# andimarafioti/faster-qwen3-tts

Measured on AMD Instinct MI355X. Metric: real-time factor (audio s / wall s), Qwen3-TTS-12Hz-0.6B voice-clone streaming chunk_size=8; p50 TTFA in ttfa_ms_p50, higher is better.
Workload: dtype bf16

## Files before the change

faster-qwen3-tts_amd/csrc/fq3_api.hip:

```cpp
#define FQ3_SKINNY_EXTERN
#include "fq3_ctx.h"
#include "sampler.cuh"
#include "sampler_wave.cuh"
#include "skinny_gemm.cuh"
#include "state_kernels.cuh"

#include <cstdio>
#include <cstdlib>
#include <cstring>
#include <map>
#include <string>
#include <type_traits>
#include <vector>

using namespace fq3;

static thread_local std::string g_err;
static int fail(int code, const std::string& m) { g_err = m; return code; }
int fq3_fail_(int code, const std::string& m) { return fail(code, m); }
#define HIPCHK(x) do { hipError_t e_ = (x); if (e_ != hipSuccess) return fail(FQ3_EHIP, std::string(#x) + ": " + hipGetErrorString(e_)); } while (0)

extern "C" const char* fq3_last_error(void) { return g_err.c_str(); }
extern "C" void fq3_set_error_(const char* msg) { g_err = msg ? msg : ""; }
extern "C" int fq3_abi_version(void) { return FQ3_ABI_VERSION; }
// ... 160 lines not shown
    };
    int r;
    {
        StackBufs& b = c->tk;
        b.max_seq = cfg->max_seq_len;
        b.max_blocks = (cfg->max_seq_len + kKeysPerTile - 1) / kKeysPerTile;
        b.workers = std::min(kMaxWorkers, b.max_blocks);
        if (!pool) {
            if ((r = pool_create_(cfg, b.max_blocks, &pool))) return r;
            pool->is_private = true;
        }
        b.pool = pool;
        { std::lock_guard<std::mutex> lk(pool->mu); ++pool->users; }
        b.k = pool->k; b.v = pool->v;
        if ((r = dmalloc(c, (void**)&b.d_table, (size_t)b.max_blocks * sizeof(int)))) return r;
        if (pool->is_private && (r = kv_ensure(c, cfg->max_seq_len, nullptr, true))) return r;
    }
    if ((r = alloc_stack(c->pk, p, pred_seq))) return r;
    const int Hm = std::max(t.hidden, p.hidden), Im = std::max(t.inter, p.inter);
    const int qkvm = std::max(t.n_heads + 2 * t.n_kv_heads, p.n_heads + 2 * p.n_kv_heads) * kHeadDim;
    const int Vm = std::max(t.vocab, p.vocab);
    const int G = cfg->num_code_groups;
    const int frames = cfg->max_frames > 0 ? cfg->max_frames : 4096;
    c->cfg.max_frames = frames;
    if ((r = dmalloc(c, &c->h, (size_t)Hm * c->esz))) return r;
    if ((r = dmalloc(c, &c->h2, (size_t)Hm * c->esz))) return r;
    if ((r = dmalloc(c, &c->qkv2, (size_t)qkvm * c->esz))) return r;
    if ((r = dmalloc(c, &c->attn_out, (size_t)qkvm * c->esz))) return r;
    if ((r = dmalloc(c, &c->attn_out2, (size_t)qkvm * c->esz))) return r;
    if ((r = dmalloc(c, &c->act2, (size_t)Im * c->esz))) return r;
    if ((r = dmalloc(c, &c->pred_x2, (size_t)p.hidden * c->esz))) return r;
    if ((r = dmalloc(c, &c->xin, (size_t)Hm * c->esz))) return r;
    if ((r = dmalloc(c, &c->tmp_hidden, (size_t)Hm * c->esz))) return r;
    if ((r = dmalloc(c, &c->qkv, (size_t)qkvm * c->esz))) return r;
    if ((r = dmalloc(c, &c->act, (size_t)Im * c->esz))) return r;
    if ((r = dmalloc(c, &c->logits, (size_t)Vm * c->esz))) return r;
    if ((r = dmalloc(c, &c->past_hidden, (size_t)t.hidden * c->esz))) return r;
    if ((r = dmalloc(c, &c->ph_hold, (size_t)t.hidden * c->esz))) return r;
    if ((r = dmalloc(c, &c->pred_in, (size_t)2 * t.hidden * c->esz))) return r;
    if ((r = dmalloc(c, &c->pred_next, (size_t)t.hidden * c->esz))) return r;
    if ((r = dmalloc(c, &c->pred_x, (size_t)p.hidden * c->esz))) return r;
    if ((r = dmalloc(c, &c->plogits, (size_t)(G - 1) * p.vocab * c->esz))) return r;
    const int maxkv = std::max(t.n_kv_heads, p.n_kv_heads);
    c->part_stride = (size_t)maxkv * kMaxWorkers * 4 * kPartStride;
    if ((r = dmalloc(c, (void**)&c->part, 2 * c->part_stride * sizeof(float)))) return r;
    if ((r = dmalloc(c, (void**)&c->rope_now, 2 * 64 * sizeof(float)))) return r;
    if ((r = dmalloc(c, (void**)&c->seen_api, kMaxVocab))) return r;
    if ((r = dmalloc(c, (void**)&c->st, sizeof(DecodeState)))) return r;
    if ((r = dmalloc(c, (void**)&c->seen, kMaxVocab))) return r;
    if ((r = dmalloc(c, (void**)&c->codes, (size_t)(frames + 1) * G * sizeof(int)))) return r;
    if ((r = dmalloc(c, (void**)&c->ids64, (size_t)64 * sizeof(int64_t)))) return r;
    if ((r = dmalloc(c, (void**)&c->d_pemb, (size_t)64 * sizeof(void*)))) return r;
    HIPCHK(hipStreamCreateWithFlags(&c->cap_stream, hipStreamNonBlocking));
    return FQ3_OK;
}

extern "C" int fq3_set_option(fq3_ctx* c, const char* key, int value) {
    if (!c || !key) return fail(FQ3_EINVAL, "null argument");
    const std::string k(key);
    if (k == "weight_nt") c->opt_nt = value;
    else if (k == "pred_m2") c->opt_m2 = value;
    else if (k == "pred_attn") c->opt_pred_attn = value;
    else if (k == "rows_per_wave_max") c->opt_rmax = value;
    else if (k == "prefill_mode") c->prefill_mode = value;
    else if (k == "flash_prefill") c->opt_flash_prefill = value;
    else if (k == "flash_small") c->opt_flash_small = value;
    else if (k == "cont_pack") c->opt_cont_pack = value;
    else if (k == "swiglu_tile") c->opt_swiglu_tile = value;
    else if (k == "packed_weights") c->opt_packed = value;
    else if (k == "skinny_gemm") c->opt_no_skinny = !value;
    else return fail(FQ3_EINVAL, "unknown option: " + k);
    fq3_graph_reset(c);
    return FQ3_OK;
}

extern "C" int fq3_graph_reset(fq3_ctx* c) {
    if (!c) return fail(FQ3_EINVAL, "null ctx");
    if (c->exec) { (void)hipGraphExecDestroy(c->exec); c->exec = nullptr; }
    if (c->graph) { (void)hipGraphDestroy(c->graph); c->graph = nullptr; }
    return FQ3_OK;
}

namespace {
struct PackedEntry { void* p; int refs; int N, K; };
std::mutex g_packed_mu;
std::map<std::pair<const void*, int>, PackedEntry> g_packed;
}
const void* fq3_packed_find_(const void* W, int kind) {
    std::lock_guard<std::mutex> lk(g_packed_mu);
    auto it = g_packed.find({W, kind});
    return it == g_packed.end() ? nullptr : it->second.p;
}
int fq3_packed_acquire_(const void* W, int N, int K, int kind) {
    if (!W || !skinny_pack_ok(N, K) || (kind == 1 && (N / 2) % 8) || (kind == 2 && N % 512)) return FQ3_EUNSUPPORTED;
    std::lock_guard<std::mutex> lk(g_packed_mu);
    auto it = g_packed.find({W, kind});
    if (it != g_packed.end()) {
        if (it->second.N != N || it->second.K != K) return fail(FQ3_EINVAL, "a matrix is bound with two different shapes");
        ++it->second.refs;
        return FQ3_OK;
    }
    void* p = nullptr;
    if (hipMalloc(&p, (size_t)N * K * 2) != hipSuccess) { (void)hipGetLastError(); return fail(FQ3_ENOMEM, "no device memory for the fragment-major weight copy"); }
    skinny_pack(reinterpret_cast<const bf16_t*>(W), reinterpret_cast<bf16_t*>(p), N, K, kind == 1 ? N / 2 : (kind == 2 ? -(N / 2) : 0), nullptr);
    if (hipStreamSynchronize(nullptr) != hipSuccess) { (void)hipFree(p); return fail(FQ3_EHIP, "packing a weight matrix failed"); }
    g_packed[{W, kind}] = PackedEntry{p, 1, N, K};
    return FQ3_OK;
}
void fq3_packed_release_(const void* W, int kind) {
    std::lock_guard<std::mutex> lk(g_packed_mu);
    auto it = g_packed.find({W, kind});
    if (it == g_packed.end()) return;
    if (--it->second.refs <= 0) { (void)hipFree(it->second.p); g_packed.erase(it); }
}
static void packed_release_all(fq3_ctx* c) {
    for (auto& r : c->packed_refs) fq3_packed_release_(r.first, r.second);
    c->packed_refs.clear();
}
static int packed_acquire_all(fq3_ctx* c) {
    if (c->cfg.dtype != FQ3_BF16) return FQ3_OK;
    auto take = [&](const void* W, int N, int K, int kind) -> int {
        const int r = fq3_packed_acquire_(W, N, K, kind);
        if (r == FQ3_OK) c->packed_refs.emplace_back(W, kind);
        return r == FQ3_EUNSUPPORTED ? FQ3_OK : r;
    };
    auto stack = [&](const std::vector<fq3_layer_weights>& L, const fq3_stack_dims& d) -> int {
        const int qd = d.n_heads * kHeadDim, kvd = d.n_kv_heads * kHeadDim;
        for (const fq3_layer_weights& l : L) {
            if (int r = take(l.qkv, qd + 2 * kvd, d.hidden, 0)) return r;
            if (int r = take(l.o, d.hidden, qd, 0)) return r;
            if (int r = take(l.gate_up, 2 * d.inter, d.hidden, 1)) return r;
            if (int r = take(l.gate_up, 2 * d.inter, d.hidden, 0)) return r;
            if (int r = take(l.down, d.hidden, d.inter, 0)) return r;
        }
        return FQ3_OK;
    };
    if (int r = stack(c->tl, c->cfg.talker)) return r;
    if (int r = stack(c->pl, c->cfg.predictor)) return r;
    for (const fq3_layer_weights& l : c->tl) if (int r = take(l.gate_up, 2 * c->cfg.talker.inter, c->cfg.talker.hidden, 2)) return r;
    if (int r = take(c->wt.codec_head, c->cfg.talker.vocab, c->cfg.talker.hidden, 0)) return r;
    for (const void* h : c->lmh) if (int r = take(h, c->cfg.predictor.vocab, c->cfg.predictor.hidden, 0)) return r;
    return FQ3_OK;
}

extern "C" int fq3_ctx_destroy(fq3_ctx* c) {
    if (!c) return FQ3_OK;
    (void)hipDeviceSynchronize();
    fq3_graph_reset(c);
    packed_release_all(c);
    if (c->cap_stream) (void)hipStreamDestroy(c->cap_stream);
    if (fq3_kv_pool* p = c->tk.pool) {
        (void)fq3_kv_release(c, 0);
        bool last;
        { std::lock_guard<std::mutex> lk(p->mu); last = --p->users == 0; }
        if (p->is_private && last) pool_free_(p);
    }
    for (void* p : c->allocs) (void)hipFree(p);
    delete c;
    return FQ3_OK;
}

extern "C" int fq3_bind_weights(fq3_ctx* c, const fq3_weight_table* w) {
    if (!c || !w) return fail(FQ3_EINVAL, "null argument");
    const int G = c->cfg.num_code_groups;
    if (!w->talker_layers || !w->predictor_layers || !w->codec_embedding || !w->codec_head || !w->talker_final_norm ||
        !w->predictor_final_norm || !w->predictor_embeddings || !w->lm_heads || !w->talker_cos || !w->talker_sin ||
        !w->pred_cos || !w->pred_sin)
        return fail(FQ3_EINVAL, "weight table has null entries");
    if (c->cfg.has_projection && !w->proj_w) return fail(FQ3_EINVAL, "has_projection set but proj_w is null");
    if (w->talker_rope_len < c->cfg.max_seq_len || w->pred_rope_len < G + 1)
        return fail(FQ3_EINVAL, "rope tables shorter than the caches");
    c->wt = *w;
    c->tl.assign(w->talker_layers, w->talker_layers + c->cfg.talker.n_layers);
    c->pl.assign(w->predictor_layers, w->predictor_layers + c->cfg.predictor.n_layers);
    c->pemb.assign(w->predictor_embeddings, w->predictor_embeddings + (G - 1));
    c->lmh.assign(w->lm_heads, w->lm_heads + (G - 1));
    for (auto& l : c->tl) if (!l.qkv || !l.o || !l.gate_up || !l.down || !l.input_norm || !l.post_norm || !l.q_norm || !l.k_norm)
        return fail(FQ3_EINVAL, "talker layer has null weights");
    for (auto& l : c->pl) if (!l.qkv || !l.o || !l.gate_up || !l.down || !l.input_norm || !l.post_norm || !l.q_norm || !l.k_norm)
        return fail(FQ3_EINVAL, "predictor layer has null weights");
    HIPCHK(hipMemcpy(c->d_pemb, c->pemb.data(), (G - 1) * sizeof(void*), hipMemcpyHostToDevice));
    (void)hipDeviceSynchronize();
    packed_release_all(c);
    if (int r = packed_acquire_all(c)) { packed_release_all(c); return r; }
    c->bound = true;
    fq3_graph_reset(c);
    return FQ3_OK;
}

template <typename T, int NCH, int PRO, int EPI, bool NT, int M = 1>
static void launch_gemv_n(const GemvArgs& a, int rmax, hipStream_t s) {
    const int R = gemv_rows_per_wave<NCH, EPI>(a.N, rmax);
    const int grid = gemv_grid(a.N, R);
    const size_t shm = gemv_lds_bytes<PRO, M>(a.K);
    if constexpr (MaxRows<NCH, EPI>::v >= 2) {
        if (R == 2) { gemv_launch<T, NCH, PRO, EPI, NT, M, 2>(a, grid, shm, s); return; }
    }
    gemv_launch<T, NCH, PRO, EPI, NT, M, 1>(a, grid, shm, s);
}
template <typename T, int PRO, int EPI>
static int launch_gemv2_t(const GemvArgs& a, int rmax, hipStream_t s) {
    constexpr int most = gemv_most_chunks(PRO, 2);
    const int n = gemv_chunks(a.K, most);
// ... 722 lines not shown
}
static int enqueue_frame(fq3_ctx* c, hipStream_t s) {
    return c->cfg.dtype == FQ3_BF16 ? enqueue_frame_t<bf16_t>(c, s) : enqueue_frame_t<float>(c, s);
}

extern "C" int fq3_graph_capture(fq3_ctx* c, void* stream) {
    NEED_BOUND(c);
    if (c->exec) return FQ3_OK;
    (void)stream;
    hipStream_t cs = c->cap_stream;
    HIPCHK(hipStreamBeginCapture(cs, hipStreamCaptureModeRelaxed));
    int r = enqueue_frame(c, cs);
    hipGraph_t g = nullptr;
    hipError_t e = hipStreamEndCapture(cs, &g);
    if (r) { if (g) (void)hipGraphDestroy(g); return r; }
    if (e != hipSuccess) return fail(FQ3_EHIP, std::string("hipStreamEndCapture: ") + hipGetErrorString(e));
    c->graph = g;
    HIPCHK(hipGraphInstantiate(&c->exec, c->graph, nullptr, nullptr, 0));
    return FQ3_OK;
}

extern "C" int fq3_decode_frames(fq3_ctx* c, int n_frames, void* stream) {
    NEED_BOUND(c);
    hipStream_t s = (hipStream_t)stream;
    for (int i = 0; i < n_frames; ++i) {
        if (c->exec) { HIPCHK(hipGraphLaunch(c->exec, s)); }
        else if (int r = enqueue_frame(c, s)) return r;
    }
    LAUNCH_CHECK();
    return FQ3_OK;
}

extern "C" int fq3_decode_poll(fq3_ctx* c, int* n_frames_total, int* done, void* stream) {
    if (!c) return fail(FQ3_EINVAL, "null ctx");
    hipStream_t s = (hipStream_t)stream;
    DecodeState h;
    HIPCHK(hipMemcpyAsync(&h, c->st, sizeof h, hipMemcpyDeviceToHost, s));
    HIPCHK(hipStreamSynchronize(s));
    if (n_frames_total) *n_frames_total = h.frame;
    if (done) *done = h.done == 2 ? 2 : (h.done || h.token == h.eos_id);
    return FQ3_OK;
}

extern "C" int fq3_decode_codes(fq3_ctx* c, int from, int count, int64_t* out, void* stream) {
    if (!c || !out) return fail(FQ3_EINVAL, "null argument");
    if (from < 0 || count < 0 || from + count > c->cfg.max_frames) return fail(FQ3_EINVAL, "range");
    const int G = c->cfg.num_code_groups, n = count * G;
    if (n == 0) return FQ3_OK;
    hipLaunchKernelGGL(codes_to_i64_kernel, dim3((n + 255) / 256), dim3(256), 0, (hipStream_t)stream,
                       c->codes + (size_t)from * G, out, n);
    LAUNCH_CHECK();
    return FQ3_OK;
}
```

faster-qwen3-tts_amd/csrc/fq3_ctx.h:

```cpp
#pragma once
#include "../../include/fq3hip.h"
#include "decode_kernels.cuh"
#include <hip/hip_runtime.h>
#include <mutex>
#include <string>
#include <utility>
#include <vector>

struct fq3_kv_pool {
    int dtype = 0, esz = 2, n_layers = 0, n_kv = 0, n_blocks = 0;
    size_t blk_elems = 0;
    std::vector<void*> k, v;
    std::vector<int> free_list;
    std::mutex mu;
    int in_use_high = 0;
    int users = 0;
    bool is_private = false;
};

struct StackBufs {
    std::vector<void*> k, v;
    int max_seq = 0, workers = 1;
    fq3_kv_pool* pool = nullptr;
    int* d_table = nullptr;
    std::vector<int> blocks;
    int max_blocks = 0;
};

struct fq3_ctx {
    fq3_config cfg{};
    int esz = 2;
    std::vector<fq3_layer_weights> tl, pl;
    fq3_weight_table wt{};
    std::vector<const void*> pemb, lmh;
    const void** d_pemb = nullptr;
    bool bound = false;
    StackBufs tk, pk;
    void *h = nullptr, *xin = nullptr, *qkv = nullptr, *act = nullptr, *logits = nullptr, *past_hidden = nullptr;
    void *pred_in = nullptr, *pred_x = nullptr, *pred_next = nullptr, *plogits = nullptr, *tmp_hidden = nullptr;
    void *attn_out = nullptr, *attn_out2 = nullptr;
    void *h2 = nullptr, *qkv2 = nullptr, *act2 = nullptr, *pred_x2 = nullptr;
    size_t part_stride = 0;
    float* part = nullptr;
    float* rope_now = nullptr;
    unsigned char* seen_api = nullptr;
    fq3::DecodeState* st = nullptr;
    fq3::TeacherForcing* tf = nullptr;
    unsigned char* seen = nullptr;
    int* codes = nullptr;
    int64_t* ids64 = nullptr;
    int n_pad = 0, rope_delta = 0;
    int opt_nt = 1;
    int opt_m2 = 1;
    int opt_pred_attn = 1;
    int opt_rmax = 2;
    int opt_flash_prefill = 1;
    int opt_flash_small = 1;
    int opt_cont_pack = 1;
    int opt_swiglu_tile = 1;
    int opt_packed = 1;
    std::vector<std::pair<const void*, int>> packed_refs;
    int opt_no_skinny = 0;
    int prefill_mode = 0;
    bool talker_wave = true;
    fq3_sampling pred_sampling{0.9f, 50, 1.0f, 1, 1.0f};
    hipGraph_t graph = nullptr;
    hipGraphExec_t exec = nullptr;
    hipStream_t cap_stream = nullptr;
    std::vector<void*> allocs;
    fq3_prompt_weights pw{};
    bool pw_bound = false;
    void *pw_x = nullptr, *pw_h = nullptr;
    int pw_cap = 0;
    void* ph_hold = nullptr;
    void *tt_tab = nullptr, *tt_x = nullptr, *tt_h = nullptr;
    int tt_alloc = 0;
    int tt_cap = 0, tt_rows = 0;
    bool tt_open = false, tt_session = false;
    bool armed = false;
    const void* begin_trailing = nullptr; int begin_trailing_len = 0;
    void *pf_x = nullptr, *pf_xn = nullptr, *pf_qkv = nullptr, *pf_att = nullptr, *pf_gu = nullptr, *pf_act = nullptr, *pf_ws = nullptr;
};


const void* fq3_packed_find_(const void* W, int kind);
int fq3_packed_acquire_(const void* W, int N, int K, int kind);
void fq3_packed_release_(const void* W, int kind);

int fq3_fail_(int code, const std::string& m);
int fq3_kv_ensure_(fq3_ctx* c, int n_pos, hipStream_t s);
int fq3_prefill_reserve_(fq3_ctx* c);
int fq3_prefill_mfma_(fq3_ctx* c, const void* embeds, int L, int n_pad, void* out_logits, void* out_hidden, hipStream_t s);
int fq3_prefill_continue_mfma_(fq3_ctx* c, const void* embeds, int start, int n, void* out_logits, void* out_hidden, hipStream_t s);
int fq3_prefill_continue_batch_mfma_(fq3_ctx* const* cs, int n, const void* const* embeds, const int* start, const int* cnt,
                                     void* const* out_logits, void* const* out_hidden, hipStream_t s);
int fq3_prefill_batch_mfma_(fq3_ctx* const* cs, int n, const void* const* embeds, const int* L, const int* n_pad, void* const* out_logits,
                            void* const* out_hidden, hipStream_t s);
int fq3_codec_head_launch_(fq3_ctx* c, const void* hidden, void* out_logits, hipStream_t s);
int fq3_dmalloc_(fq3_ctx* c, void** p, size_t bytes);
void fq3_text_project_launch_(fq3_ctx* c, const int64_t* ids, int n, void* x, void* h, void* out, hipStream_t s);
```

faster-qwen3-tts_amd/csrc/state_kernels.cuh:

```cuda
#pragma once
#include "batch_kernels.cuh"

namespace fq3 {

static __global__ void poll_gather_kernel(LaneSt t, int B, int* out) {
    const int l = threadIdx.x;
    if (l < B) {
        const DecodeState* st = t.st[l];
        out[2 * l] = st->frame;
        out[2 * l + 1] = st->done == 2 ? 2 : ((st->done || st->token == st->eos_id) ? 1 : 0);
    }
}

struct AppendDst { void* dst[kMaxLanes]; int first[kMaxLanes + 1]; };
struct AppendPub { DecodeState* st[kMaxLanes]; int rows[kMaxLanes]; int closes[kMaxLanes]; };
static __global__ __launch_bounds__(256) void text_scatter_kernel(AppendDst a, int n_items, const u32x4* y, int row_vec) {
    const int r = blockIdx.x;
    int lo = 0, hi = n_items - 1;
    while (lo < hi) {
        const int mid = (lo + hi + 1) >> 1;
        if (a.first[mid] <= r) lo = mid; else hi = mid - 1;
    }
    u32x4* d = gptr(reinterpret_cast<u32x4*>(a.dst[lo])) + (size_t)(r - a.first[lo]) * row_vec;
    const u32x4* src = y + (size_t)r * row_vec;
    for (int e = threadIdx.x; e < row_vec; e += 256) d[e] = src[e];
}
static __global__ __launch_bounds__(kMaxLanes) void text_publish_lanes_kernel(AppendPub p, int n_items) {
    const int i = threadIdx.x;
    if (i < n_items) {
        DecodeState* st = gptr(p.st[i]);
        st->trailing_len = p.rows[i];
        if (p.closes[i]) st->text_open = 0;
    }
}

struct KvTableVals { int v[128]; };
static __global__ void kv_table_write_kernel(int* table, KvTableVals vals, int first, int count) {
    const int i = threadIdx.x;
    if (i < count) table[first + i] = vals.v[i];
}

template <typename T, bool TO_CACHE>
__global__ __launch_bounds__(256) void kv_paged_copy_kernel(T* cache, const int* table, int blk_stride, T* dense, int n_kv, int L) {
    constexpr int EPC = 16 / (int)sizeof(T), CPR = kHeadDim / EPC;
    const int i = blockIdx.x * 256 + threadIdx.x;
    if (i >= n_kv * L * CPR) return;
    const int ch = i % CPR, row = i / CPR, key = row % L, h = row / L;
    T* cp = cache + (size_t)table[key / kKeysPerTile] * blk_stride + ((size_t)h * kKeysPerTile + key % kKeysPerTile) * kHeadDim + ch * EPC;
    T* dp = dense + ((size_t)h * L + key) * kHeadDim + ch * EPC;
    if (TO_CACHE) *reinterpret_cast<u32x4*>(cp) = *reinterpret_cast<const u32x4*>(dp);
    else *reinterpret_cast<u32x4*>(dp) = *reinterpret_cast<const u32x4*>(cp);
}

struct KvAdoptTab { void* dst[128]; const void* src[128]; };
template <typename T>
__global__ __launch_bounds__(256) void kv_adopt_kernel(KvAdoptTab t, const int* dst_table, const int* src_table, int blk_elems) {
    const int which = blockIdx.x, b = blockIdx.y;
    const u32x4* s = reinterpret_cast<const u32x4*>(reinterpret_cast<const T*>(t.src[which]) + (size_t)src_table[b] * blk_elems);
    u32x4* d = reinterpret_cast<u32x4*>(reinterpret_cast<T*>(t.dst[which]) + (size_t)dst_table[b] * blk_elems);
    const int n16 = blk_elems * (int)sizeof(T) / 16;
    for (int i = threadIdx.x; i < n16; i += 256) d[i] = s[i];
}

static __global__ __launch_bounds__(256) void decode_arm_kernel(DecodeState* st, DecodeState init, unsigned char* seen, int seen_bytes,
                                                                uint32_t* past_hidden, const uint32_t* ph_src, int ph_words) {
    for (int i = threadIdx.x; i < seen_bytes / 4; i += 256) reinterpret_cast<uint32_t*>(seen)[i] = 0u;
    for (int i = threadIdx.x; i < ph_words; i += 256) past_hidden[i] = ph_src[i];
    if (threadIdx.x == 0) *st = init;
}
static __global__ void decode_set_forced_kernel(TeacherForcing* tf, const int* forced, int* decisions) {
    tf->forced = forced; tf->decisions = decisions;
}
static __global__ void decode_cancel_kernel(DecodeState* st) { st->done = 1; }
static __global__ void codes_to_i64_kernel(const int* src, int64_t* dst, int n) {
    const int i = blockIdx.x * blockDim.x + threadIdx.x;
    if (i < n) dst[i] = src[i];
}

}
```

faster-qwen3-tts_amd/fq3hip/_lib.py:

```python
from __future__ import annotations

import ctypes as C
import os

import torch

_HERE = os.path.dirname(os.path.abspath(__file__))
LIB_PATH = os.path.join(os.path.dirname(_HERE), "lib", "libfq3hip.so")

FQ3_BF16, FQ3_F32, FQ3_BF16X2 = 0, 1, 2
FQ3_PCM_F32, FQ3_PCM_S16, FQ3_PCM_MULAW, FQ3_PCM_ALAW = 0, 1, 2, 3
FQ3_STAGE_GROUP_MAX = 32
FQ3_OK, FQ3_EINVAL, FQ3_EHIP, FQ3_ESTATE, FQ3_ETOOLONG, FQ3_EUNSUPPORTED, FQ3_ENOMEM = 0, -1, -2, -3, -4, -5, -6

vp = C.c_void_p
i32 = C.c_int32


class StackDims(C.Structure):
    _fields_ = [("hidden", i32), ("inter", i32), ("n_layers", i32), ("n_heads", i32), ("n_kv_heads", i32),
                ("head_dim", i32), ("vocab", i32), ("rms_eps", C.c_float)]


class Config(C.Structure):
# ... 78 lines not shown


class RefEncConfig(C.Structure):
    _fields_ = [("num_filters", i32), ("n_ratios", i32), ("ratios", i32 * 8), ("kernel_size", i32), ("last_kernel_size", i32),
                ("residual_kernel_size", i32), ("n_residual_layers", i32), ("dilation_growth_rate", i32), ("compress", i32),
                ("hidden", i32), ("n_layers", i32), ("n_heads", i32), ("head_dim", i32), ("inter", i32), ("sliding_window", i32),
                ("norm_eps", C.c_float), ("num_quantizers", i32), ("num_semantic", i32), ("codebook_size", i32),
                ("codebook_dim", i32), ("max_positions", i32), ("mel_dim", i32), ("n_fft", i32), ("hop", i32),
                ("n_bins_padded", i32), ("n_enc", i32), ("enc_channels", i32 * 8), ("enc_kernel_sizes", i32 * 8),
                ("enc_dilations", i32 * 8), ("attn_channels", i32), ("res2net_scale", i32), ("se_channels", i32),
                ("enc_dim", i32)]


SIGNATURES = {
    "fq3_last_error": (C.c_char_p, []),
    "fq3_abi_version": (C.c_int, []),
    "fq3_ctx_create": (C.c_int, [C.POINTER(Config), C.POINTER(vp)]),
    "fq3_ctx_destroy": (C.c_int, [vp]),
    "fq3_kv_pool_create": (C.c_int, [C.POINTER(Config), C.c_int, C.POINTER(vp)]),
    "fq3_kv_pool_destroy": (C.c_int, [vp]),
    "fq3_kv_pool_stats": (C.c_int, [vp, C.POINTER(C.c_int), C.POINTER(C.c_int), C.POINTER(C.c_int), C.POINTER(C.c_int64)]),
    "fq3_ctx_create_pooled": (C.c_int, [C.POINTER(Config), vp, C.POINTER(vp)]),
    "fq3_kv_reserve": (C.c_int, [vp, C.c_int, vp]),
    "fq3_kv_release": (C.c_int, [vp, C.c_int]),
    "fq3_kv_blocks": (C.c_int, [vp]),
    "fq3_bind_weights": (C.c_int, [vp, C.POINTER(WeightTable)]),
    "fq3_set_option": (C.c_int, [vp, C.c_char_p, C.c_int]),
    "fq3_kv_import": (C.c_int, [vp, C.c_int, vp, vp, C.c_int, vp]),
    "fq3_kv_export": (C.c_int, [vp, C.c_int, vp, vp, C.c_int, vp]),
    "fq3_kv_adopt": (C.c_int, [vp, vp, C.c_int, vp]),
    "fq3_kv_copy": (C.c_int, [vp, vp, C.c_int, vp]),
    "fq3_set_generation_state": (C.c_int, [vp, C.c_int, C.c_int]),
    "fq3_talker_step": (C.c_int, [vp, vp, C.c_int, vp, vp]),
    "fq3_prefill": (C.c_int, [vp, vp, C.c_int, C.c_int, vp, vp, vp]),
    "fq3_prefill_continue": (C.c_int, [vp, vp, C.c_int, C.c_int, vp, vp, vp]),
    "fq3_prefill_reserve": (C.c_int, [vp]),
    "fq3_prefill_continue_batch": (C.c_int, [C.POINTER(vp), C.c_int, C.POINTER(vp), C.POINTER(C.c_int), C.POINTER(C.c_int), C.POINTER(vp),
                                             C.POINTER(vp), vp]),
    "fq3_prefill_batch": (C.c_int, [C.POINTER(vp), C.c_int, C.POINTER(vp), C.POINTER(C.c_int), C.POINTER(C.c_int), C.POINTER(vp),
                                    C.POINTER(vp), vp]),
    "fq3_set_prefill_mode": (C.c_int, [vp, C.c_int]),
    "fq3_codec_head": (C.c_int, [vp, vp, vp, vp]),
    "fq3_set_predictor_sampling": (C.c_int, [vp, C.POINTER(Sampling)]),
    "fq3_predictor_loop": (C.c_int, [vp, vp, vp, vp, vp, vp]),
    "fq3_sample": (C.c_int, [vp, vp, C.c_int, C.POINTER(Sampling), vp, C.c_int, C.c_int, C.c_int, C.c_int,
                             C.c_int, vp, vp, vp]),
    "fq3_apply_repetition_penalty": (C.c_int, [vp, vp, C.c_int, vp, C.c_int, C.c_float, vp]),
    "fq3_decode_begin": (C.c_int, [vp, C.POINTER(DecodeParams), vp]),
    "fq3_decode_cancel": (C.c_int, [vp, vp]),
    "fq3_decode_set_forced": (C.c_int, [vp, vp, vp, vp]),
    "fq3_decode_frames": (C.c_int, [vp, C.c_int, vp]),
    "fq3_decode_poll": (C.c_int, [vp, C.POINTER(C.c_int), C.POINTER(C.c_int), vp]),
    "fq3_decode_codes": (C.c_int, [vp, C.c_int, C.c_int, vp, vp]),
    "fq3_graph_capture": (C.c_int, [vp, vp]),
    "fq3_graph_reset": (C.c_int, [vp]),
    "fq3_bind_prompt_weights": (C.c_int, [vp, C.POINTER(PromptWeights)]),
    "fq3_text_project": (C.c_int, [vp, vp, C.c_int, vp, vp]),
    "fq3_decode_text_open": (C.c_int, [vp, C.c_int, vp]),
    "fq3_decode_text_append": (C.c_int, [vp, vp, C.c_int, C.c_int, vp]),
    "fq3_decode_text_rows": (C.c_int, [vp, C.POINTER(C.c_int), C.POINTER(C.c_int)]),
    "fq3_decode_text_read": (C.c_int, [vp, C.c_int, C.c_int, vp, vp]),
    "fq3_prompt_rows": (C.c_int, [vp, vp, C.c_int, vp, C.c_int, vp, C.c_int, vp, vp, vp]),
    "fq3_batch_create": (C.c_int, [C.POINTER(vp), C.c_int, C.POINTER(vp)]),
    "fq3_batch_destroy": (C.c_int, [vp]),
    "fq3_batch_size": (C.c_int, [vp]),
    "fq3_batch_frames": (C.c_int, [vp, C.c_int, vp]),
    "fq3_batch_graph_capture": (C.c_int, [vp, vp]),
    "fq3_batch_graph_reset": (C.c_int, [vp]),
    "fq3_batch_set_option": (C.c_int, [vp, C.c_char_p, C.c_int]),
    "fq3_batch_set_group_streams": (C.c_int, [vp, C.POINTER(vp), C.c_int]),
    "fq3_batch_poll_async": (C.c_int, [vp, C.c_int, vp]),
    "fq3_batch_poll_wait": (C.c_int, [vp, C.c_int, C.POINTER(C.c_int), C.POINTER(C.c_int)]),
    "fq3_batch_text_append": (C.c_int, [vp, C.c_int, C.POINTER(C.c_int32), C.POINTER(C.c_int32), C.POINTER(C.c_int32), vp, vp]),
    "fq3_codec_create": (C.c_int, [C.POINTER(CodecConfig), C.POINTER(vp)]),
    "fq3_codec_destroy": (C.c_int, [vp]),
    "fq3_codec_set_option": (C.c_int, [vp, C.c_char_p, C.c_int]),
    "fq3_codec_bind": (C.c_int, [vp, C.c_char_p, vp, C.c_int64]),
    "fq3_codec_finalize": (C.c_int, [vp, vp]),
    "fq3_codec_num_samples": (C.c_int64, [vp, C.c_int]),
    "fq3_codec_decode": (C.c_int, [vp, vp, C.c_int, vp, vp]),
    "fq3_codec_decode_tail": (C.c_int, [vp, vp, C.c_int, C.c_int64, vp, vp]),
    "fq3_codec_decode_batch": (C.c_int, [vp, vp, C.c_int, C.c_int, C.c_int64, vp, vp]),
    "fq3_codec_prefix_create": (C.c_int, [vp, vp, C.c_int, C.POINTER(vp), vp]),
    "fq3_codec_prefix_destroy": (C.c_int, [vp]),
    "fq3_codec_prefix_frames": (C.c_int, [vp]),
    "fq3_codec_decode_batch_prefix": (C.c_int, [vp, C.POINTER(vp), vp, C.c_int, C.c_int, C.c_int64, vp, vp]),
    "fq3_codec_stream_create": (C.c_int, [vp, vp, C.POINTER(vp), vp]),
    "fq3_codec_stream_reset": (C.c_int, [vp, vp, vp]),
    "fq3_codec_stream_destroy": (C.c_int, [vp]),
    "fq3_codec_stream_frames": (C.c_int, [vp]),
    "fq3_codec_stream_push": (C.c_int, [vp, C.POINTER(vp), C.c_int, vp, C.c_int, vp, vp]),
    "fq3_refenc_create": (C.c_int, [C.POINTER(RefEncConfig), C.POINTER(vp)]),
    "fq3_refenc_destroy": (C.c_int, [vp]),
    "fq3_refenc_bind": (C.c_int, [vp, C.c_char_p, vp, C.c_int64]),
    "fq3_refenc_finalize": (C.c_int, [vp, vp]),
    "fq3_refenc_num_frames": (C.c_int64, [vp, C.c_int64]),
    "fq3_refenc_encode": (C.c_int, [vp, vp, C.c_int64, vp, vp]),
    "fq3_refenc_speaker": (C.c_int, [vp, vp, C.c_int64, vp, vp, vp]),
    "fq3_audio_out_design": (C.c_int, [C.c_int, C.c_int, C.c_int, C.POINTER(C.c_int), C.POINTER(C.c_int), C.POINTER(C.c_int),
                                       C.POINTER(C.c_float), C.c_int64]),
    "fq3_audio_out_count": (C.c_int64, [C.c_int, C.c_int, C.c_int, C.c_int64, C.c_int]),
    "fq3_audio_out_create": (C.c_int, [C.POINTER(AudioOutConfig), C.POINTER(vp)]),
    "fq3_audio_out_destroy": (C.c_int, [vp]),
    "fq3_audio_out_reset": (C.c_int, [vp, vp]),
    "fq3_audio_out_push": (C.c_int, [vp, vp, C.c_int64, C.c_int, vp, C.c_int64, C.POINTER(C.c_int64), vp]),
    "fq3_tsm_design": (C.c_int, [C.c_int, C.c_int, C.POINTER(C.c_int), C.POINTER(C.c_int), C.POINTER(C.c_int),
# ... 80 lines not shown
```

faster-qwen3-tts_amd/fq3hip/engine.py:

```python
from __future__ import annotations

import ctypes as C
import threading
from typing import Dict, Optional

import torch

from . import _lib as L
from .config import TTSConfig, StackConfig

Weights = Dict[str, torch.Tensor]
_CAPTURE_LOCK = threading.Lock()


def _ptr(t: Optional[torch.Tensor]) -> Optional[int]:
    return None if t is None else t.data_ptr()


def rope_tables(head_dim: int, theta: float, n_pos: int, dtype: torch.dtype):
    inv = 1.0 / (theta ** (torch.arange(0, head_dim, 2, dtype=torch.float) / head_dim))
    ang = torch.arange(n_pos, dtype=torch.float32)[:, None] * inv[None, :]
    return ang.cos().to(dtype).float().contiguous(), ang.sin().to(dtype).float().contiguous()


# ... 429 lines not shown
        self._loop_keep = (past_hidden, trailing_text, tts_pad_embed, talker_noise, pred_noise)
        L.check(self.lib.fq3_decode_begin(self.ctx, C.byref(p), self._stream()))

    def graph_capture(self):
        with _CAPTURE_LOCK:
            L.check(self.lib.fq3_graph_capture(self.ctx, self._stream()))

    def graph_reset(self):
        L.check(self.lib.fq3_graph_reset(self.ctx))

    def decode_frames(self, n: int):
        L.check(self.lib.fq3_decode_frames(self.ctx, int(n), self._stream()))

    def decode_poll(self):
        n, d = C.c_int(0), C.c_int(0)
        L.check(self.lib.fq3_decode_poll(self.ctx, C.byref(n), C.byref(d), self._stream()))
        return n.value, bool(d.value)

    def decode_poll_state(self):
        n, d = C.c_int(0), C.c_int(0)
        L.check(self.lib.fq3_decode_poll(self.ctx, C.byref(n), C.byref(d), self._stream()))
        return n.value, int(d.value)

    def decode_text_open(self, capacity_rows: int):
        L.check(self.lib.fq3_decode_text_open(self.ctx, int(capacity_rows), self._stream()))

    def decode_text_append(self, ids, final: bool = False):
        if isinstance(ids, torch.Tensor):
            t = ids.reshape(-1).to(device=self.device, dtype=torch.long).contiguous()
        else:
            t = torch.tensor([int(i) for i in ids], dtype=torch.long, device=self.device)
        n = int(t.numel())
        L.check(self.lib.fq3_decode_text_append(self.ctx, t.data_ptr() if n else None, n, int(bool(final)), self._stream()))
        self._text_ids_keep = t

    def decode_text_rows(self):
        n, c = C.c_int(0), C.c_int(0)
        L.check(self.lib.fq3_decode_text_rows(self.ctx, C.byref(n), C.byref(c)))
        return n.value, bool(c.value)

    def decode_text_read(self, start: int = 0, count: Optional[int] = None) -> torch.Tensor:
        if count is None:
            count = self.decode_text_rows()[0] - int(start)
        out = self.new(int(count), self.cfg.talker.hidden_size)
        L.check(self.lib.fq3_decode_text_read(self.ctx, int(start), int(count), out.data_ptr(), self._stream()))
        return out

    def decode_codes(self, start: int, count: int) -> torch.Tensor:
        out = torch.empty(count, self.cfg.num_code_groups, dtype=torch.long, device=self.device)
        if count:
            L.check(self.lib.fq3_decode_codes(self.ctx, int(start), int(count), out.data_ptr(), self._stream()))
        return out

    def close(self):
        if getattr(self, "ctx", None) and self.ctx.value:
            self.lib.fq3_ctx_destroy(self.ctx)
            self.ctx = L.vp()

    def __del__(self):
        try:
            self.close()
        except Exception:
            pass


class Fq3Batch:

    def __init__(self, lanes):
        lanes = list(lanes)
        if not 1 <= len(lanes) <= 128:
            raise ValueError("a batch holds 1..128 lanes")
        self.lanes = lanes
        self.lib = lanes[0].lib
        self.device = lanes[0].device
        arr = (L.vp * len(lanes))(*[e.ctx.value for e in lanes])
        self.handle = L.vp()
        with torch.cuda.device(self.device):
            L.check(self.lib.fq3_batch_create(arr, len(lanes), C.byref(self.handle)))

    def __len__(self):
        return len(self.lanes)

    def _stream(self) -> int:
        return torch.cuda.current_stream(self.device).cuda_stream

    def frames(self, n: int):
        L.check(self.lib.fq3_batch_frames(self.handle, int(n), self._stream()))

    def graph_capture(self):
        with _CAPTURE_LOCK:
            L.check(self.lib.fq3_batch_graph_capture(self.handle, self._stream()))

    def graph_reset(self):
        L.check(self.lib.fq3_batch_graph_reset(self.handle))

    def set_option(self, key: str, value: int):
        L.check(self.lib.fq3_batch_set_option(self.handle, key.encode(), int(value)))

    def poll_async(self, slot: int):
        L.check(self.lib.fq3_batch_poll_async(self.handle, int(slot), self._stream()))

    def poll_wait(self, slot: int):
        n = len(self.lanes)
        a, d = (C.c_int * n)(), (C.c_int * n)()
        L.check(self.lib.fq3_batch_poll_wait(self.handle, int(slot), a, d))
        return list(a), [bool(x) for x in d]
# ... 37 lines not shown
```

faster-qwen3-tts_amd/fq3hip/generate.py:

```python
from __future__ import annotations

import numbers
import time
from typing import Optional, Tuple

import torch

from .predictor_graph import PredictorGraph
from .talker_graph import TalkerGraph

NOISE_RING = 64


def validate_seed(seed):
    if seed is None:
        return None
    if isinstance(seed, bool) or not isinstance(seed, numbers.Integral):
        raise ValueError(f"seed must be an integer in [0, 2**64) or None, got {type(seed).__name__}")
    seed = int(seed)
    if not 0 <= seed < 2 ** 64:
        raise ValueError(f"seed must be in [0, 2**64), got {seed}")
    return seed


def expand_seeds(seeds, n: int):
    if seeds is None:
        return [None] * n
    if isinstance(seeds, (list, tuple)):
        if len(seeds) != n:
            raise ValueError(f"seeds: {len(seeds)} entries for {n} utterances")
        return [validate_seed(s) for s in seeds]
    s = validate_seed(seeds)
    return [(s + i) % 2 ** 64 for i in range(n)]


def _refill(engine, talker_noise, pred_noise, seed=None, first_frame=0):
    if seed is not None:
        if talker_noise is not None or pred_noise is not None:
            engine.noise_fill(talker_noise, pred_noise, seed, first_frame)
        return
    if talker_noise is not None:
        talker_noise.exponential_(1)
    if pred_noise is not None:
        pred_noise.exponential_(1)


def _first_noise(eng, V, do_sample, seed):
    if not do_sample:
        return None
    if seed is not None:
        return eng.noise_first(seed)
    return torch.empty(V, dtype=eng.dtype, device=eng.device).exponential_(1)


def _n_pad_of(attention_mask) -> int:
    if attention_mask is None:
        return 0
    known = noted_n_pad(attention_mask)
    return known if known is not None else int((attention_mask[0] == 0).sum())


def noted_n_pad(attention_mask):
    note = getattr(attention_mask, "fq3_n_pad", None)
    if not (isinstance(note, tuple) and len(note) == 2):
# ... 86 lines not shown
                     trailing_text=tth, tts_pad_embed=tpe, temperature=temperature, top_k=top_k, top_p=top_p,
                     do_sample=do_sample, repetition_penalty=repetition_penalty, min_new_tokens=min_new_tokens,
                     max_new_tokens=max_frames, talker_noise=tn, pred_noise=pn, noise_frames=NOISE_RING)
    if use_graph:
        eng.graph_capture()
    else:
        eng.graph_reset()
    return eng, tn, pn, max_frames


def _prefill_and_arm(talker, talker_input_embeds, attention_mask, trailing_text_hiddens, tts_pad_embed, config,
                     predictor_graph, talker_graph, max_new_tokens, min_new_tokens, temperature, top_k, top_p,
                     do_sample, repetition_penalty, use_graph, cache=None, seed=None):
    token, hidden, n_rows, n_pad = _prefill_first_token(talker_graph.engine, talker_input_embeds, attention_mask, config,
                                                        min_new_tokens, temperature, top_k, top_p, do_sample, cache=cache, seed=seed)
    return _arm_decode(talker, config, token, hidden, n_rows, attention_mask, trailing_text_hiddens, tts_pad_embed, predictor_graph,
                       talker_graph, max_new_tokens, min_new_tokens, temperature, top_k, top_p, do_sample, repetition_penalty,
                       use_graph, n_pad=n_pad, seed=seed)


def run_frames(eng, tn, pn, issued: int, count: int, seed=None):
    while count > 0:
        if issued % NOISE_RING == 0:
            if seed is None:
                _refill(eng, tn, pn)
            else:
                _refill(eng, tn, pn, seed, issued)
        k = min(count, NOISE_RING - issued % NOISE_RING)
        eng.decode_frames(k)
        issued += k
        count -= k
    return issued


@torch.inference_mode()
def fast_generate(talker, talker_input_embeds: torch.Tensor, attention_mask: torch.Tensor,
                  trailing_text_hiddens: torch.Tensor, tts_pad_embed: torch.Tensor, config,
                  predictor_graph: PredictorGraph, talker_graph: TalkerGraph, max_new_tokens: int = 2048,
                  min_new_tokens: int = 2, temperature: float = 0.9, top_k: int = 50, top_p: float = 1.0,
                  do_sample: bool = True, repetition_penalty: float = 1.05,
                  subtalker_dosample: Optional[bool] = None, subtalker_top_k: Optional[int] = None,
                  subtalker_top_p: Optional[float] = None, subtalker_temperature: Optional[float] = None,
                  parity_mode: bool = False, poll_every: int = 8, seed: Optional[int] = None) -> Tuple[Optional[torch.Tensor], dict]:
    seed = validate_seed(seed)
    t_start = time.time()
    eng, tn, pn, max_frames = _prefill_and_arm(
        talker, talker_input_embeds, attention_mask, trailing_text_hiddens, tts_pad_embed, config, predictor_graph,
        talker_graph, max_new_tokens, min_new_tokens, temperature, top_k, top_p, do_sample, repetition_penalty,
        use_graph=not parity_mode, seed=seed)
    torch.cuda.current_stream(eng.device).synchronize()
    t_prefill = time.time() - t_start
    t_decode_start = time.time()
    issued, n, done = 0, 0, False
    while not done and issued < max_frames:
        issued = run_frames(eng, tn, pn, issued, min(poll_every, max_frames - issued), seed)
        n, done = eng.decode_poll()
    codes = eng.decode_codes(0, n) if n > 0 else None
    torch.cuda.current_stream(eng.device).synchronize()
    t_decode = time.time() - t_decode_start
    timing = {
        "prefill_ms": t_prefill * 1000,
        "decode_s": t_decode,
        "steps": n,
        "ms_per_step": (t_decode / n * 1000) if n > 0 else 0,
        "steps_per_s": (n / t_decode) if t_decode > 0 else 0,
    }
    return codes, timing
```

faster-qwen3-tts_amd/fq3hip/streaming.py:

```python
from __future__ import annotations

import time
from typing import Generator, Tuple

import torch

from .generate import _prefill_and_arm, run_frames, validate_seed
from .predictor_graph import PredictorGraph
from .talker_graph import TalkerGraph


@torch.inference_mode()
def fast_generate_streaming(talker, talker_input_embeds: torch.Tensor, attention_mask: torch.Tensor,
                            trailing_text_hiddens: torch.Tensor, tts_pad_embed: torch.Tensor, config,
                            predictor_graph: PredictorGraph, talker_graph: TalkerGraph, max_new_tokens: int = 2048,
                            min_new_tokens: int = 2, temperature: float = 0.9, top_k: int = 50, top_p: float = 1.0,
                            do_sample: bool = True, repetition_penalty: float = 1.05, chunk_size: int = 12,
                            use_graph: bool = True, seed=None) -> Generator[Tuple[torch.Tensor, dict], None, None]:
    seed = validate_seed(seed)
    t_start = time.time()
    eng, tn, pn, max_frames = _prefill_and_arm(
        talker, talker_input_embeds, attention_mask, trailing_text_hiddens, tts_pad_embed, config, predictor_graph,
        talker_graph, max_new_tokens, min_new_tokens, temperature, top_k, top_p, do_sample, repetition_penalty,
        use_graph=use_graph, seed=seed)
    torch.cuda.current_stream(eng.device).synchronize()
    t_prefill = time.time() - t_start
    issued, emitted, chunk_count, done = 0, 0, 0, False
    chunk_start = time.time()
    issued = run_frames(eng, tn, pn, issued, min(chunk_size, max_frames), seed)
    while True:
        n, done = eng.decode_poll()
        new = n - emitted
        if new <= 0:
            break
        chunk = eng.decode_codes(emitted, new)
        ready = torch.cuda.Event()
        ready.record(torch.cuda.current_stream(eng.device))
        emitted = n
        is_final = new < chunk_size
        more = (not done) and (not is_final) and issued < max_frames
        if more:
            issued = run_frames(eng, tn, pn, issued, min(chunk_size, max_frames - issued), seed)
        yield chunk, {
            "chunk_index": chunk_count,
            "chunk_steps": new,
            "prefill_ms": t_prefill * 1000 if chunk_count == 0 else 0,
            "decode_ms": (time.time() - chunk_start) * 1000,
            "total_steps_so_far": emitted,
            "is_final": is_final,
            "codes_ready_event": ready,
        }
        chunk_count += 1
        chunk_start = time.time()
        if not more:
            break


def parity_generate_streaming(talker, talker_input_embeds, attention_mask, trailing_text_hiddens, tts_pad_embed, config,
                              max_new_tokens: int = 2048, min_new_tokens: int = 2, temperature: float = 0.9,
                              top_k: int = 50, top_p: float = 1.0, do_sample: bool = True,
                              repetition_penalty: float = 1.05, chunk_size: int = 12, predictor_graph=None,
                              talker_graph=None, seed=None):
    if predictor_graph is None or talker_graph is None:
        raise ValueError("parity_generate_streaming needs the graph objects of the HIP context")
    return fast_generate_streaming(talker, talker_input_embeds, attention_mask, trailing_text_hiddens, tts_pad_embed,
                                   config, predictor_graph, talker_graph, max_new_tokens=max_new_tokens,
                                   min_new_tokens=min_new_tokens, temperature=temperature, top_k=top_k, top_p=top_p,
                                   do_sample=do_sample, repetition_penalty=repetition_penalty, chunk_size=chunk_size,
                                   use_graph=False, seed=seed)
```

include/fq3hip.h:

```cpp
#ifndef FQ3HIP_H
#define FQ3HIP_H

#include <stdint.h>

#ifdef __cplusplus
extern "C" {
#endif

#define FQ3_ABI_VERSION 5

enum { FQ3_BF16 = 0, FQ3_F32 = 1,
       FQ3_BF16X2 = 2 };
enum { FQ3_OK = 0, FQ3_EINVAL = -1, FQ3_EHIP = -2, FQ3_ESTATE = -3, FQ3_ETOOLONG = -4, FQ3_EUNSUPPORTED = -5, FQ3_ENOMEM = -6 };

typedef struct fq3_stack_dims {
    int32_t hidden, inter, n_layers, n_heads, n_kv_heads, head_dim, vocab;
    float rms_eps;
} fq3_stack_dims;

typedef struct fq3_config {
    int32_t dtype;
    fq3_stack_dims talker;
    fq3_stack_dims predictor;
    int32_t num_code_groups;
// ... 71 lines not shown

int fq3_prefill(fq3_ctx* ctx, const void* embeds, int L, int n_pad, void* out_logits, void* out_hidden,
                void* stream);
int fq3_prefill_continue(fq3_ctx* ctx, const void* embeds, int start, int n, void* out_logits, void* out_hidden, void* stream);
int fq3_prefill_batch(fq3_ctx* const* ctxs, int n, const void* const* embeds, const int* L, const int* n_pad,
                      void* const* out_logits, void* const* out_hidden, void* stream);

int fq3_prefill_continue_batch(fq3_ctx* const* ctxs, int n, const void* const* embeds, const int* start, const int* cnt,
                               void* const* out_logits, void* const* out_hidden, void* stream);

int fq3_prefill_reserve(fq3_ctx* ctx);

int fq3_set_prefill_mode(fq3_ctx* ctx, int mode);

int fq3_codec_head(fq3_ctx* ctx, const void* hidden, void* out_logits, void* stream);


int fq3_set_predictor_sampling(fq3_ctx* ctx, const fq3_sampling* s);

int fq3_predictor_loop(fq3_ctx* ctx, const void* pred_input, const void* noise, int64_t* out_ids,
                       void* out_logits, void* stream);


int fq3_sample(fq3_ctx* ctx, const void* logits, int V, const fq3_sampling* s, const int64_t* history,
               int n_hist, int sup_lo, int sup_hi, int keep_id, int suppress_eos, const void* noise,
               int64_t* out_token, void* stream);

int fq3_apply_repetition_penalty(fq3_ctx* ctx, void* logits, int V, const int64_t* history, int n_hist, float penalty,
                                 void* stream);


typedef struct fq3_decode_params {
    fq3_sampling talker;
    int32_t min_new_tokens;
    int32_t max_new_tokens;
    int32_t prefill_len;
    int32_t gen_step;
    int32_t first_token;
    const void* past_hidden;
    const void* trailing_text;
    int32_t trailing_len;
    const void* tts_pad_embed;
    const void* talker_noise;
    const void* pred_noise;
    int32_t noise_frames;
} fq3_decode_params;

int fq3_decode_begin(fq3_ctx* ctx, const fq3_decode_params* p, void* stream);
int fq3_decode_cancel(fq3_ctx* ctx, void* stream);
int fq3_decode_set_forced(fq3_ctx* ctx, const int32_t* forced_codes, int32_t* decisions, void* stream);
int fq3_decode_frames(fq3_ctx* ctx, int n_frames, void* stream);
int fq3_decode_poll(fq3_ctx* ctx, int* n_frames_total, int* done, void* stream);
int fq3_decode_codes(fq3_ctx* ctx, int from, int count, int64_t* out_codes_dev, void* stream);
int fq3_graph_capture(fq3_ctx* ctx, void* stream);
int fq3_graph_reset(fq3_ctx* ctx);

typedef struct fq3_prompt_weights {
    const void* text_embedding;
    const void* fc1_w;
    const void* fc1_b;
    const void* fc2_w;
    const void* fc2_b;
    int32_t text_vocab, text_hidden;
} fq3_prompt_weights;
int fq3_bind_prompt_weights(fq3_ctx* ctx, const fq3_prompt_weights* w);
int fq3_text_project(fq3_ctx* ctx, const int64_t* ids, int n, void* out, void* stream);
int fq3_prompt_rows(fq3_ctx* ctx, const void* text_rows, int n_text, const int32_t* prog, int n_rows,
                    const int64_t* ref_codes, int n_ref, const void* spk_embed, void* out, void* stream);

int fq3_decode_text_open(fq3_ctx* ctx, int capacity_rows, void* stream);
int fq3_decode_text_append(fq3_ctx* ctx, const int64_t* ids, int n, int final, void* stream);
int fq3_decode_text_rows(const fq3_ctx* ctx, int* n_rows, int* closed);
int fq3_decode_text_read(fq3_ctx* ctx, int from, int count, void* out, void* stream);

typedef struct fq3_batch fq3_batch;
int fq3_batch_create(fq3_ctx* const* lanes, int n_lanes, fq3_batch** out);
int fq3_batch_destroy(fq3_batch* b);
int fq3_batch_size(const fq3_batch* b);
int fq3_batch_frames(fq3_batch* b, int n_frames, void* stream);
int fq3_batch_graph_capture(fq3_batch* b, void* stream);
int fq3_batch_graph_reset(fq3_batch* b);
int fq3_batch_poll_async(fq3_batch* b, int slot, void* stream);
int fq3_batch_poll_wait(fq3_batch* b, int slot, int* n_frames_total, int* done);
int fq3_batch_text_append(fq3_batch* b, int n_items, const int32_t* lane, const int32_t* count, const int32_t* final_,
                          const int64_t* ids, void* stream);
int fq3_batch_set_option(fq3_batch* b, const char* key, int value);
int fq3_batch_set_group_streams(fq3_batch* b, void* const* streams, int n);

typedef struct fq3_codec fq3_codec;
typedef struct fq3_codec_config {
    int32_t dtype;
    int32_t codebook_size, codebook_dim, rvq_dim, num_quantizers, num_semantic;
    int32_t latent_dim, hidden, inter, n_layers, n_heads, head_dim, sliding_window;
    float rms_eps;
    int32_t n_upsample;  int32_t upsampling_ratios[4];
    int32_t n_rates;     int32_t upsample_rates[8];
    int32_t decoder_dim;
    int32_t max_frames;
} fq3_codec_config;
int fq3_codec_create(const fq3_codec_config* cfg, fq3_codec** out);
int fq3_codec_destroy(fq3_codec* c);
int fq3_codec_bind(fq3_codec* c, const char* name, const void* ptr, int64_t numel);
int fq3_codec_set_option(fq3_codec* codec, const char* key, int value);
int fq3_codec_finalize(fq3_codec* c, void* stream);
int64_t fq3_codec_num_samples(const fq3_codec* c, int T);
int fq3_codec_decode(fq3_codec* c, const int64_t* codes, int T, float* pcm, void* stream);
// ... 131 lines not shown
```

Before: 38.93.

## Pipeline decode polling with event marks and lookahead frame issue

After: 39.29, median of 6. About the same (+0.9%).

```diff
diff --git a/faster-qwen3-tts_amd/csrc/fq3_api.hip b/faster-qwen3-tts_amd/csrc/fq3_api.hip
--- a/faster-qwen3-tts_amd/csrc/fq3_api.hip
+++ b/faster-qwen3-tts_amd/csrc/fq3_api.hip
@@ -236,6 +236,9 @@
     if ((r = dmalloc(c, (void**)&c->ids64, (size_t)64 * sizeof(int64_t)))) return r;
     if ((r = dmalloc(c, (void**)&c->d_pemb, (size_t)64 * sizeof(void*)))) return r;
     HIPCHK(hipStreamCreateWithFlags(&c->cap_stream, hipStreamNonBlocking));
+    if ((r = dmalloc(c, (void**)&c->mark_dev, (size_t)kMarkSlots * 2 * sizeof(int)))) return r;
+    HIPCHK(hipHostMalloc((void**)&c->mark_host, (size_t)kMarkSlots * 2 * sizeof(int), hipHostMallocDefault));
+    for (int i = 0; i < kMarkSlots; ++i) HIPCHK(hipEventCreateWithFlags(&c->mark_ev[i], hipEventDisableTiming));
     return FQ3_OK;
 }
 
@@ -333,6 +336,8 @@
     fq3_graph_reset(c);
     packed_release_all(c);
     if (c->cap_stream) (void)hipStreamDestroy(c->cap_stream);
+    for (int i = 0; i < kMarkSlots; ++i) if (c->mark_ev[i]) (void)hipEventDestroy(c->mark_ev[i]);
+    if (c->mark_host) (void)hipHostFree(c->mark_host);
     if (fq3_kv_pool* p = c->tk.pool) {
         (void)fq3_kv_release(c, 0);
         bool last;
@@ -1161,3 +1166,30 @@
     LAUNCH_CHECK();
     return FQ3_OK;
 }
+
+extern "C" int fq3_decode_mark(fq3_ctx* c, int slot, int from, int count, int64_t* out, void* stream) {
+    NEED_BOUND(c);
+    if (slot < 0 || slot >= kMarkSlots) return fail(FQ3_EINVAL, "mark slot must be 0..3");
+    if (from < 0 || count < 0 || from > c->cfg.max_frames - count) return fail(FQ3_EINVAL, "range");
+    hipStream_t s = (hipStream_t)stream;
+    const int G = c->cfg.num_code_groups, n = out ? count * G : 0;
+    int* d = c->mark_dev + 2 * slot;
+    hipLaunchKernelGGL(decode_mark_kernel, dim3(n > 0 ? (n + 255) / 256 : 1), dim3(256), 0, s, (const DecodeState*)c->st, d,
+                       (const int*)(c->codes + (size_t)from * G), out ? out + (size_t)from * G : nullptr, n, from, G);
+    LAUNCH_CHECK();
+    HIPCHK(hipMemcpyAsync(c->mark_host + 2 * slot, d, 2 * sizeof(int), hipMemcpyDeviceToHost, s));
+    HIPCHK(hipEventRecord(c->mark_ev[slot], s));
+    c->mark_armed[slot] = true;
+    return FQ3_OK;
+}
+
+extern "C" int fq3_decode_mark_wait(fq3_ctx* c, int slot, int* n_frames_total, int* done) {
+    NEED_BOUND(c);
+    if (slot < 0 || slot >= kMarkSlots) return fail(FQ3_EINVAL, "mark slot must be 0..3");
+    if (!c->mark_armed[slot]) return fail(FQ3_ESTATE, "no mark is queued in this slot");
+    HIPCHK(hipEventSynchronize(c->mark_ev[slot]));
+    c->mark_armed[slot] = false;
+    if (n_frames_total) *n_frames_total = c->mark_host[2 * slot];
+    if (done) *done = c->mark_host[2 * slot + 1];
+    return FQ3_OK;
+}
diff --git a/faster-qwen3-tts_amd/csrc/fq3_ctx.h b/faster-qwen3-tts_amd/csrc/fq3_ctx.h
--- a/faster-qwen3-tts_amd/csrc/fq3_ctx.h
+++ b/faster-qwen3-tts_amd/csrc/fq3_ctx.h
@@ -26,6 +26,8 @@
     std::vector<int> blocks;
     int max_blocks = 0;
 };
+
+constexpr int kMarkSlots = 4;
 
 struct fq3_ctx {
     fq3_config cfg{};
@@ -79,6 +81,10 @@
     bool tt_open = false, tt_session = false;
     bool armed = false;
     const void* begin_trailing = nullptr; int begin_trailing_len = 0;
+    int* mark_dev = nullptr;
+    int* mark_host = nullptr;
+    hipEvent_t mark_ev[kMarkSlots] = {};
+    bool mark_armed[kMarkSlots] = {};
     void *pf_x = nullptr, *pf_xn = nullptr, *pf_qkv = nullptr, *pf_att = nullptr, *pf_gu = nullptr, *pf_act = nullptr, *pf_ws = nullptr;
 };
 
diff --git a/faster-qwen3-tts_amd/csrc/state_kernels.cuh b/faster-qwen3-tts_amd/csrc/state_kernels.cuh
--- a/faster-qwen3-tts_amd/csrc/state_kernels.cuh
+++ b/faster-qwen3-tts_amd/csrc/state_kernels.cuh
@@ -76,5 +76,14 @@
     const int i = blockIdx.x * blockDim.x + threadIdx.x;
     if (i < n) dst[i] = src[i];
 }
+static __global__ void decode_mark_kernel(const DecodeState* st, int* mark, const int* src, int64_t* dst, int n, int from, int G) {
+    const int i = blockIdx.x * blockDim.x + threadIdx.x;
+    const int frame = st->frame;
+    if (i == 0) {
+        mark[0] = frame;
+        mark[1] = st->done == 2 ? 2 : ((st->done || st->token == st->eos_id) ? 1 : 0);
+    }
+    if (dst && i < min(n, (frame - from) * G)) dst[i] = src[i];
+}
 
 }
diff --git a/faster-qwen3-tts_amd/fq3hip/_lib.py b/faster-qwen3-tts_amd/fq3hip/_lib.py
--- a/faster-qwen3-tts_amd/fq3hip/_lib.py
+++ b/faster-qwen3-tts_amd/fq3hip/_lib.py
@@ -154,6 +154,8 @@
     "fq3_decode_frames": (C.c_int, [vp, C.c_int, vp]),
     "fq3_decode_poll": (C.c_int, [vp, C.POINTER(C.c_int), C.POINTER(C.c_int), vp]),
     "fq3_decode_codes": (C.c_int, [vp, C.c_int, C.c_int, vp, vp]),
+    "fq3_decode_mark": (C.c_int, [vp, C.c_int, C.c_int, C.c_int, vp, vp]),
+    "fq3_decode_mark_wait": (C.c_int, [vp, C.c_int, C.POINTER(C.c_int), C.POINTER(C.c_int)]),
     "fq3_graph_capture": (C.c_int, [vp, vp]),
     "fq3_graph_reset": (C.c_int, [vp]),
     "fq3_bind_prompt_weights": (C.c_int, [vp, C.POINTER(PromptWeights)]),
diff --git a/faster-qwen3-tts_amd/fq3hip/engine.py b/faster-qwen3-tts_amd/fq3hip/engine.py
--- a/faster-qwen3-tts_amd/fq3hip/engine.py
+++ b/faster-qwen3-tts_amd/fq3hip/engine.py
@@ -505,6 +505,20 @@
             L.check(self.lib.fq3_decode_codes(self.ctx, int(start), int(count), out.data_ptr(), self._stream()))
         return out
 
+    def decode_mark(self, slot: int, start: int, count: int, out: Optional[torch.Tensor] = None):
+        if out is not None:
+            G = self.cfg.num_code_groups
+            if (out.dtype != torch.long or not out.is_contiguous() or out.device.type != "cuda" or out.dim() != 2 or out.shape[1] != G
+                    or int(start) < 0 or int(count) < 0 or out.shape[0] < int(start) + int(count)):
+                raise ValueError(f"decode_mark out: need a contiguous device LongTensor[>= {int(start) + int(count)}, {G}], got "
+                                 f"{out.dtype} {tuple(out.shape)} on {out.device}")
+        L.check(self.lib.fq3_decode_mark(self.ctx, int(slot), int(start), int(count), _ptr(out), self._stream()))
+
+    def decode_mark_wait(self, slot: int):
+        n, d = C.c_int(0), C.c_int(0)
+        L.check(self.lib.fq3_decode_mark_wait(self.ctx, int(slot), C.byref(n), C.byref(d)))
+        return n.value, bool(d.value)
+
     def close(self):
         if getattr(self, "ctx", None) and self.ctx.value:
             self.lib.fq3_ctx_destroy(self.ctx)
diff --git a/faster-qwen3-tts_amd/fq3hip/generate.py b/faster-qwen3-tts_amd/fq3hip/generate.py
--- a/faster-qwen3-tts_amd/fq3hip/generate.py
+++ b/faster-qwen3-tts_amd/fq3hip/generate.py
@@ -10,6 +10,8 @@
 from .talker_graph import TalkerGraph
 
 NOISE_RING = 64
+MARK_SLOTS = 4
+MARK_LOOKAHEAD = 2
 
 
 def validate_seed(seed):
@@ -202,6 +204,15 @@
     t_prefill = time.time() - t_start
     t_decode_start = time.time()
     issued, n, done = 0, 0, False
+    if hasattr(eng, "decode_mark") and hasattr(eng, "decode_mark_wait"):
+        ahead, marked, k = min(MARK_LOOKAHEAD, poll_every), 0, 0
+        while not done and marked < max_frames:
+            marked = min(marked + poll_every, max_frames)
+            issued = run_frames(eng, tn, pn, issued, marked - issued, seed)
+            eng.decode_mark(k % MARK_SLOTS, 0, 0)
+            issued = run_frames(eng, tn, pn, issued, min(ahead, max_frames - issued), seed)
+            n, done = eng.decode_mark_wait(k % MARK_SLOTS)
+            k += 1
     while not done and issued < max_frames:
         issued = run_frames(eng, tn, pn, issued, min(poll_every, max_frames - issued), seed)
         n, done = eng.decode_poll()
diff --git a/faster-qwen3-tts_amd/fq3hip/streaming.py b/faster-qwen3-tts_amd/fq3hip/streaming.py
--- a/faster-qwen3-tts_amd/fq3hip/streaming.py
+++ b/faster-qwen3-tts_amd/fq3hip/streaming.py
@@ -5,7 +5,7 @@
 
 import torch
 
-from .generate import _prefill_and_arm, run_frames, validate_seed
+from .generate import MARK_SLOTS, _prefill_and_arm, run_frames, validate_seed
 from .predictor_graph import PredictorGraph
 from .talker_graph import TalkerGraph
 
@@ -16,7 +16,8 @@
                             predictor_graph: PredictorGraph, talker_graph: TalkerGraph, max_new_tokens: int = 2048,
                             min_new_tokens: int = 2, temperature: float = 0.9, top_k: int = 50, top_p: float = 1.0,
                             do_sample: bool = True, repetition_penalty: float = 1.05, chunk_size: int = 12,
-                            use_graph: bool = True, seed=None) -> Generator[Tuple[torch.Tensor, dict], None, None]:
+                            use_graph: bool = True, seed=None,
+                            lookahead: int = 2) -> Generator[Tuple[torch.Tensor, dict], None, None]:
     seed = validate_seed(seed)
     t_start = time.time()
     eng, tn, pn, max_frames = _prefill_and_arm(
@@ -27,6 +28,42 @@
     t_prefill = time.time() - t_start
     issued, emitted, chunk_count, done = 0, 0, 0, False
     chunk_start = time.time()
+    if hasattr(eng, "decode_mark") and hasattr(eng, "decode_mark_wait"):
+        ahead = max(0, min(int(lookahead), chunk_size))
+        codes = torch.empty(max_frames, eng.cfg.num_code_groups, dtype=torch.long, device=eng.device)
+        ready = torch.cuda.Event()
+        ready.record(torch.cuda.current_stream(eng.device))
+        issued = marked = run_frames(eng, tn, pn, issued, min(chunk_size, max_frames), seed)
+        eng.decode_mark(0, 0, marked, codes)
+        issued = run_frames(eng, tn, pn, issued, min(ahead, max_frames - issued), seed)
+        while True:
+            n, done = eng.decode_mark_wait(chunk_count % MARK_SLOTS)
+            new = n - emitted
+            if new <= 0:
+                break
+            chunk = codes[emitted:n]
+            emitted = n
+            is_final = new < chunk_size
+            more = (not done) and (not is_final) and marked < max_frames
+            if more:
+                marked = min(marked + chunk_size, max_frames)
+                issued = run_frames(eng, tn, pn, issued, marked - issued, seed)
+                eng.decode_mark((chunk_count + 1) % MARK_SLOTS, emitted, marked - emitted, codes)
+                issued = run_frames(eng, tn, pn, issued, min(ahead, max_frames - issued), seed)
+            yield chunk, {
+                "chunk_index": chunk_count,
+                "chunk_steps": new,
+                "prefill_ms": t_prefill * 1000 if chunk_count == 0 else 0,
+                "decode_ms": (time.time() - chunk_start) * 1000,
+                "total_steps_so_far": emitted,
+                "is_final": is_final,
+                "codes_ready_event": ready,
+            }
+            chunk_count += 1
+            chunk_start = time.time()
+            if not more:
+                break
+        return
     issued = run_frames(eng, tn, pn, issued, min(chunk_size, max_frames), seed)
     while True:
         n, done = eng.decode_poll()
diff --git a/include/fq3hip.h b/include/fq3hip.h
--- a/include/fq3hip.h
+++ b/include/fq3hip.h
@@ -147,6 +147,8 @@
 int fq3_decode_frames(fq3_ctx* ctx, int n_frames, void* stream);
 int fq3_decode_poll(fq3_ctx* ctx, int* n_frames_total, int* done, void* stream);
 int fq3_decode_codes(fq3_ctx* ctx, int from, int count, int64_t* out_codes_dev, void* stream);
+int fq3_decode_mark(fq3_ctx* ctx, int slot, int from, int count, int64_t* out_codes_dev, void* stream);
+int fq3_decode_mark_wait(fq3_ctx* ctx, int slot, int* n_frames_total, int* done);
 int fq3_graph_capture(fq3_ctx* ctx, void* stream);
 int fq3_graph_reset(fq3_ctx* ctx);
 
```
